# bitlayer-org/tap-stark

Hardware: AMD Instinct MI355X
Metric: trace cells/sec (proofs/sec alongside), 2^20x64 BabyBear trace (higher is better)
Workload: dtype u32

## Files before the change

### tap-stark_amd/csrc/kernels.hpp

```cpp
#pragma once
#include <stdint.h>

#include "bb.hpp"
#include "context.hpp"
#include "ntt_plan.hpp"

namespace ts {

struct ColMat {
    uint32_t* d = nullptr;
    uint64_t height = 0;
    uint32_t width = 0;
    uint64_t col_stride = 0;
};

void launch_build_twiddles(Context& ctx, uint32_t* W, uint32_t* Winv, unsigned log_size);
void launch_build_shift_tables(Context& ctx, uint32_t* lo, uint32_t* hi, uint32_t n_hi,
                               uint32_t n_cosets, uint32_t shift_mont, unsigned log_N,
                               unsigned log_blowup, uint32_t scale_mont);
const uint32_t* coset_scale_table(Context& ctx, unsigned log_n, unsigned log_blowup, uint32_t shift);
void launch_transpose_bitrev(Context& ctx, const uint32_t* src, uint32_t* dst, unsigned log_n,
                             uint32_t w, uint64_t dst_col_stride, uint32_t src_width = 0);
bool launch_transpose_bitrev_r16(Context& ctx, const uint32_t* src, uint32_t* dst, unsigned log_n, uint32_t w,
                                 uint64_t dst_col_stride, uint32_t src_width = 0);
void launch_transpose_plain(Context& ctx, const uint32_t* src, uint32_t* dst, uint64_t n, uint32_t w,
                            uint64_t dst_col_stride);
void launch_transpose_to_row_major(Context& ctx, const uint32_t* src, uint64_t col_stride,
                                   uint32_t* dst, uint64_t h, uint32_t w);
void launch_transpose_unbitrev(Context& ctx, const uint32_t* src, uint64_t col_stride, uint32_t* dst,
                               unsigned log_h, uint32_t w);
void coset_lde(Context& ctx, uint32_t* evals, uint64_t in_col_stride, uint32_t ncols, unsigned log_n,
               unsigned log_blowup, uint32_t shift, uint32_t* out, uint64_t out_col_stride,
               uint32_t beta0 = 0, uint32_t n_beta = 0, bool first_round_done = false,
               uint32_t* evals2 = nullptr, uint32_t shift2 = 0, uint32_t gw = 0, bool stage_timers = true);

inline void ntt_require_shape(const NttPlan& p, uint32_t ncols, uint64_t stride_a, uint64_t stride_b, bool lde) {
    if (const char* why = ntt_plan_refusal(p, ncols, stride_a, stride_b, lde)) throw Error(TS_ERR_INVALID, why);
}
void launch_contig_inverse(Context& ctx, const NttPlan& p, uint32_t* data, uint64_t col_stride, uint32_t ncols,
                           bool first_round_done = false, uint32_t* data2 = nullptr, uint32_t gw = 0xffffffffu);
void launch_contig_forward(Context& ctx, const NttPlan& p, uint32_t* data, uint64_t col_stride, uint32_t ncols,
                           uint32_t n_blocks);

void dft_columns(Context& ctx, uint32_t* cols, uint64_t col_stride, uint32_t ncols, unsigned log_n, bool inverse,
                 uint32_t shift);
void dft_batch(Context& ctx, const uint32_t* in, uint32_t* out, unsigned log_n, uint32_t w, bool inverse,
               uint32_t shift);
void coset_lde_batch(Context& ctx, const uint32_t* in, uint32_t* out, unsigned log_n, uint32_t w, unsigned added_bits,
                     uint32_t shift, bool bit_reversed);
void launch_bit_reverse_rows(Context& ctx, const uint32_t* src, uint32_t* dst, unsigned log_h, uint32_t w);

constexpr int MAX_BATCH_MATS = 64;
struct LeafMats {
    const uint32_t* d[MAX_BATCH_MATS];
    uint64_t col_stride[MAX_BATCH_MATS];
    uint32_t width[MAX_BATCH_MATS];
    uint8_t row_shift[MAX_BATCH_MATS];
    uint32_t n_mats;
    uint32_t total_width;
    const uint32_t* const* cols;
};
void launch_leaf_hash(Context& ctx, const LeafMats& mats, uint64_t height, uint32_t* digests);
void launch_leaf_hash_ef_pairs(Context& ctx, const uint32_t* vec, uint64_t n_rows, uint32_t* digests);
struct DevChallenger;
bool launch_merkle_levels(Context& ctx, uint32_t* tree, unsigned log_leaves,
                          DevChallenger* ch = nullptr, uint32_t* root_out = nullptr,
                          Ef* beta_out = nullptr);
void launch_merkle_tree_from(Context& ctx, uint32_t* tree, unsigned log_leaves, unsigned first_level,
                             DevChallenger* ch, uint32_t* root_out, Ef* beta_out);
bool leaf_tree_enabled(unsigned log_leaves);
void launch_commit_tree(Context& ctx, const LeafMats& mats, unsigned log_leaves, uint32_t* tree,
                        uint32_t* root_out = nullptr);
void launch_shard_top(Context& ctx, const uint32_t* subroots, uint32_t G, uint32_t* top,
                      DevChallenger* ch, uint32_t* root_out, Ef* beta_out);
void launch_merkle_one_level(Context& ctx, const uint32_t* children, uint32_t* parents,
                             uint64_t n_parents);
void launch_merkle_inject(Context& ctx, uint32_t* nodes, const uint32_t* inj, uint64_t n);
inline uint64_t merkle_level_offset(unsigned log_leaves, unsigned level) {
    uint64_t off = 0;
    for (unsigned l = 0; l < level; l++) off += (uint64_t)1 << (log_leaves - l);
    return off;
}
inline uint64_t merkle_total_digests(unsigned log_leaves) { return ((uint64_t)2 << log_leaves) - 1; }

struct AirProgram;
const uint32_t* selector_table(Context& ctx, unsigned log_n, unsigned log_qd, uint32_t shift);
constexpr int MAX_QUOTIENT_CHUNKS = 64;
struct QuotOut {
    uint32_t* chunk[MAX_QUOTIENT_CHUNKS];
};
void launch_quotient(Context& ctx, const AirProgram& air, const ColMat& trace_lde, unsigned log_n,
                     unsigned log_qd, const uint32_t* d_consts_mont, const uint32_t* d_alpha_pows_mont,
                     const QuotOut& out, uint64_t row_begin = 0, uint64_t row_end = 0,
                     uint32_t shift = GENERATOR, const ColMat* prep_lde = nullptr);
void launch_chunk_mix(Context& ctx, uint32_t* const* d_chunk_ptrs, uint32_t qd, uint64_t rows, uint64_t col_stride,
                      const uint32_t* d_mix_mont);

void launch_check_constraints(Context& ctx, const AirProgram& air, const uint32_t* trace_row_major,
                              uint64_t n, const uint32_t* d_consts_mont,
                              unsigned long long* d_violation, const uint32_t* prep_row_major = nullptr);

void launch_bary_weights(Context& ctx, unsigned log_n, const Ef* points_mont, uint32_t n_points,
                         Ef* out, uint32_t coset_gen = 0);
struct BaryPending {
    DevBuf<uint32_t> partial[3];
    uint32_t* out[3] = {nullptr, nullptr, nullptr};
    uint32_t n_blocks[3] = {0, 0, 0}, n_words[3] = {0, 0, 0};
    uint32_t n = 0, capacity = 2;
};
void launch_bary_dots(Context& ctx, const ColMat& m, unsigned log_n, const Ef* weights,
                      uint32_t n_points, Ef* out, BaryPending* pending = nullptr);
void launch_bary_finish(Context& ctx, BaryPending& pending);
struct ReduceArgs {
    Ef z_mont[2];
    Ef off_mont[2];
    Ef rys[2];
    uint32_t n_points;
    uint32_t accumulate;
};
void launch_reduce(Context& ctx, const ColMat& m, unsigned log_h, const uint32_t* d_alpha_pows_mont,
                   const ReduceArgs& args, Ef* ro);
struct FusedReduceArgs {
    Ef z_mont[2];
    Ef off_t[2];
    Ef k0, k1;
    const uint32_t* chunk_w;
    const uint32_t* chunk[MAX_QUOTIENT_CHUNKS];
    uint64_t chunk_stride;
    uint32_t n_chunks;
    uint64_t row0, rows;
};
void launch_reduce_fused(Context& ctx, const ColMat& trace, unsigned log_h,
                         const uint32_t* d_alpha_pows_mont, const FusedReduceArgs& args, Ef* ro,
                         const ColMat* prep = nullptr, const Ef* prep_off_mont = nullptr);
void launch_reduce_low(Context& ctx, const ColMat& trace, unsigned log_n, const uint32_t* d_alpha_pows_mont,
                       const FusedReduceArgs& args, const Ef* weights, uint32_t* out);
void launch_ef_interleave(Context& ctx, const uint32_t* cols, uint64_t col_stride, uint64_t rows, Ef* out);

void launch_fri_fold(Context& ctx, const Ef* in, uint64_t h, Ef beta_canonical, Ef* out,
                     uint32_t* next_digests);
void launch_fri_fold_dev(Context& ctx, const Ef* in, uint64_t h, const Ef* d_beta, Ef* out,
                         uint32_t* next_digests, uint64_t h_global = 0, uint64_t row0 = 0);
struct FriRoundLaunch {
    const Ef* prev = nullptr;
    const Ef* d_beta_prev = nullptr;
    Ef* cur = nullptr;
    uint64_t h = 0;
    uint32_t* tree = nullptr;
    DevChallenger* ch = nullptr;
    uint32_t* root_out = nullptr;
    Ef* beta_out = nullptr;
    uint64_t h_global = 0, row0 = 0;
};
void launch_fri_commit_round(Context& ctx, const FriRoundLaunch& r);
constexpr int FRI_TAIL_LOG = 10;
constexpr uint32_t FRI_POW_NONE = 0xffffffffu;
void launch_fri_tail(Context& ctx, const Ef* in, uint32_t L0, uint32_t blowup, DevChallenger* ch,
                     Ef* tail_vecs, uint32_t* tail_trees, uint32_t* roots_out, Ef* betas_out,
                     Ef* final_out, uint32_t pow_bits = 0, uint32_t* pow_out = nullptr,
                     const Ef* beta_in = nullptr);
void launch_vec_add(Context& ctx, Ef* acc, const Ef* other, uint64_t n);
struct FriGatherDesc {
    const uint32_t* vec;
    const uint32_t* tree;
    uint32_t log_leaves;
    uint32_t shift;
    uint64_t out_vals;
    uint64_t out_path;
};
struct RowGatherJob {
    LeafMats mats;
    uint32_t shift;
    uint32_t pad;
    uint64_t out;
};
void launch_gather_queries(Context& ctx, const RowGatherJob* d_rows, uint32_t n_rows, uint32_t max_row_width,
                           const FriGatherDesc* d_descs, uint32_t n_descs, uint32_t max_log_leaves,
                           const uint32_t* d_indices, uint32_t n_idx, uint32_t* out);

double alu_ceiling(Context& ctx, int kind);
double bench_stage(Context& ctx, int stage, unsigned log_n, uint32_t width, unsigned log_blowup, uint32_t reps);

void launch_trace_fibonacci(Context& ctx, uint32_t* out, uint32_t a, uint32_t b, uint64_t n);
void launch_trace_synth_mul(Context& ctx, uint32_t* out, uint64_t n, uint32_t width, uint64_t seed);
void launch_trace_synth_ext(Context& ctx, uint32_t* out, uint64_t n, uint32_t width, uint64_t seed);

enum : uint8_t { COL_U32 = 0, COL_U16 = 1, COL_U8 = 2, COL_MONTY32 = 3, COL_MONTY31 = 4 };
struct IngestPlan {
    bool planar = false;
    uint64_t height = 0;
    uint32_t width = 0;
    uint64_t stride = 0;
    uint64_t bytes = 0;
    int uniform4 = -1;
    std::vector<uint64_t> table;
};
IngestPlan ingest_plan(const uint8_t* kinds, uint32_t n_kinds, bool planar, uint64_t row_stride, uint64_t height,
                       uint32_t width);
void launch_ingest(Context& ctx, const IngestPlan& plan, const uint8_t* src, uint32_t* out);
void launch_scale_words(Context& ctx, const uint32_t* in, uint32_t* out, uint64_t n, uint32_t mult);
uint32_t monty_ingest_factor(uint32_t kind);

}
```

### tap-stark_amd/csrc/ntt_dft.hip

```cpp
#include <algorithm>

#include "ntt_rounds.hpp"

namespace ts {

constexpr int DFT_LO_BITS = 10;

__device__ __forceinline__ uint32_t dft_factor(const uint32_t* __restrict__ lo, const uint32_t* __restrict__ hi,
                                               uint32_t k) {
    return mont_mul(lo[k & ((1u << DFT_LO_BITS) - 1)], hi[k >> DFT_LO_BITS]);
}

template <bool INV, bool SCALE, int PLAN, int TILE = TILE_ELEMS, int NTM = NT_MID>
__global__ void __launch_bounds__(NTM)
k_dft_mid(uint32_t* data, uint64_t col_stride, unsigned log_len, unsigned log_T, unsigned row_shift,
          const uint32_t* __restrict__ W, const uint32_t* __restrict__ f_lo, const uint32_t* __restrict__ f_hi) {
    __shared__ uint32_t s[padded(TILE)];
    constexpr int PER_THREAD = TILE / NTM;
    if (PLAN == 1) {
        log_len = 8;
        log_T = 5;
    }
    const uint32_t j2_0 = blockIdx.x << log_T;
    uint32_t* g = data + (uint64_t)blockIdx.y * col_stride + j2_0;
    const uint32_t total = 1u << (log_len + log_T);
    const uint32_t tmask = (1u << log_T) - 1;
    auto off = [&](uint32_t i) { return ((i >> log_T) << row_shift) + (i & tmask); };
    if constexpr (PLAN == 1) {
        uint32_t t[PER_THREAD];
#pragma unroll
        for (int k = 0; k < PER_THREAD; k++) t[k] = g[off(threadIdx.x + (uint32_t)k * NTM)];
#pragma unroll
        for (int k = 0; k < PER_THREAD; k++) {
            const uint32_t i = threadIdx.x + (uint32_t)k * NTM;
            if (!INV && SCALE) t[k] = mont_mul_lazy(t[k], dft_factor(f_lo, f_hi, off(i) + j2_0));
            s[pad(i)] = t[k];
        }
    } else {
        for (uint32_t i = threadIdx.x; i < total; i += NTM) {
            uint32_t v = g[off(i)];
            if (!INV && SCALE) v = mont_mul_lazy(v, dft_factor(f_lo, f_hi, off(i) + j2_0));
            s[pad(i)] = v;
        }
    }
    __syncthreads();
    if constexpr (PLAN == 1) {
        if (!INV) {
            radix_round<4, false, 9, NTM, true>(s, 13, 0, 0, 0, W);
            radix_round<4, false, 5, NTM>(s, 13, 4, 0, 0, W);
        } else {
            radix_round<4, true, 5, NTM>(s, 13, 4, 0, 0, W);
            radix_round<4, true, 9, NTM, true>(s, 13, 0, 0, 0, W);
        }
    } else {
        if (!INV) tile_forward_rt<NTM>(s, log_len, log_T, 0, 0, W);
        else tile_inverse_rt<NTM>(s, log_len, log_T, 0, 0, W);
    }
    auto finish = [&](uint32_t v, uint32_t i) {
        if (INV) return SCALE ? mont_mul(v, dft_factor(f_lo, f_hi, off(i) + j2_0)) : red2p(v);
        return row_shift != 0 ? v : red2p(v);
    };
    if constexpr (PLAN == 1) {
        uint32_t t[PER_THREAD];
#pragma unroll
        for (int k = 0; k < PER_THREAD; k++) t[k] = s[pad(threadIdx.x + (uint32_t)k * NTM)];
#pragma unroll
        for (int k = 0; k < PER_THREAD; k++) {
            const uint32_t i = threadIdx.x + (uint32_t)k * NTM;
            g[off(i)] = finish(t[k], i);
        }
    } else {
        for (uint32_t i = threadIdx.x; i < total; i += NTM) g[off(i)] = finish(s[pad(i)], i);
    }
}

__global__ void __launch_bounds__(256)
k_bit_reverse_rows(const uint32_t* __restrict__ src, uint32_t* __restrict__ dst, unsigned log_h, uint32_t w) {
    const uint64_t idx = ((uint64_t)blockIdx.y * gridDim.x + blockIdx.x) * 256 + threadIdx.x;
    const uint64_t r = idx / w;
    if (r >> log_h) return;
    const uint32_t c = (uint32_t)(idx - r * w);
    dst[idx] = src[(uint64_t)bitrev32((uint32_t)r, log_h) * w + c];
}

void launch_bit_reverse_rows(Context& ctx, const uint32_t* src, uint32_t* dst, unsigned log_h, uint32_t w) {
    const uint64_t blocks = ((((uint64_t)w) << log_h) + 255) / 256;
    const uint32_t gx = (uint32_t)std::min<uint64_t>(blocks, 1u << 20);
    TS_LAUNCH(ctx, k_bit_reverse_rows, dim3(gx, (uint32_t)((blocks + gx - 1) / gx)), dim3(256), 0, src, dst, log_h, w);
    TS_HIP(hipGetLastError());
}

template <bool INV, bool SCALE>
static void launch_dft_mid_of(Context& ctx, const NttPlan& p, uint32_t* cols, uint64_t col_stride, uint32_t ncols,
                              const uint32_t* f_lo, const uint32_t* f_hi, const char* const (&names)[3]) {
    const uint32_t* W = INV ? ctx.d_twiddle_inv : ctx.d_twiddle_fwd;
    auto launch = [&](auto kernel) {
        TS_LAUNCH_NAMED(ctx, names[(int)p.mid], kernel, dim3(p.tiles, ncols), dim3(NT_MID), 0, cols, col_stride,
                        p.log_len, p.log_T, p.row_shift, W, f_lo, f_hi);
    };
    if (p.mid == NttMid::TILE16384) launch(k_dft_mid<INV, SCALE, 0, 16384>);
    else if (p.mid == NttMid::FIXED256) launch(k_dft_mid<INV, SCALE, 1>);
    else launch(k_dft_mid<INV, SCALE, 0>);
}

static void launch_dft_mid(Context& ctx, const NttPlan& p, uint32_t* cols, uint64_t col_stride, uint32_t ncols,
                           bool inverse, bool scale, const uint32_t* f_lo, const uint32_t* f_hi) {
    if (inverse)
        launch_dft_mid_of<true, true>(ctx, p, cols, col_stride, ncols, f_lo, f_hi,
                                      {"(k_dft_mid<true, true, 0>)", "(k_dft_mid<true, true, 1>)",
                                       "(k_dft_mid<true, true, 0, 16384>)"});
    else if (scale)
        launch_dft_mid_of<false, true>(ctx, p, cols, col_stride, ncols, f_lo, f_hi,
                                       {"(k_dft_mid<false, true, 0>)", "(k_dft_mid<false, true, 1>)",
                                        "(k_dft_mid<false, true, 0, 16384>)"});
    else
        launch_dft_mid_of<false, false>(ctx, p, cols, col_stride, ncols, f_lo, f_hi,
                                        {"(k_dft_mid<false, false, 0>)", "(k_dft_mid<false, false, 1>)",
                                         "(k_dft_mid<false, false, 0, 16384>)"});
}

void dft_columns(Context& ctx, uint32_t* cols, uint64_t col_stride, uint32_t ncols, unsigned log_n, bool inverse,
                 uint32_t shift) {
    if (ncols == 0) return;
    TS_REQUIRE(shift != 0 && shift < P, TS_ERR_INVALID, "dft: the coset shift must be in [1, p)");
    const NttPlan p = ntt_plan(log_n);
    ntt_require_shape(p, ncols, col_stride, 0, false);
    ctx.ensure_twiddles(log_n == 0 ? 1 : log_n);

    const bool scale = inverse || shift != 1;
    DevBuf<uint32_t> lo, hi;
    if (scale) {
        const uint32_t n_hi = log_n > (unsigned)DFT_LO_BITS ? 1u << (log_n - DFT_LO_BITS) : 1u;
        lo = DevBuf<uint32_t>(&ctx, 1u << DFT_LO_BITS);
        hi = DevBuf<uint32_t>(&ctx, n_hi);
        const uint32_t n_inv = inv_canon((uint32_t)((1ull << log_n) % P));
        launch_build_shift_tables(ctx, lo.p, hi.p, n_hi, 1, to_mont(inverse ? inv_canon(shift) : shift), log_n, 0,
                                  inverse ? to_mont(n_inv) : R_MOD_P);
    }
    if (inverse) {
        if (p.two_pass) launch_contig_inverse(ctx, p, cols, col_stride, ncols);
        launch_dft_mid(ctx, p, cols, col_stride, ncols, true, true, lo.p, hi.p);
    } else {
        launch_dft_mid(ctx, p, cols, col_stride, ncols, false, scale, lo.p, hi.p);
        if (p.two_pass) launch_contig_forward(ctx, p, cols, col_stride, ncols, 1);
    }
    TS_HIP(hipGetLastError());
}

void dft_batch(Context& ctx, const uint32_t* in, uint32_t* out, unsigned log_n, uint32_t w, bool inverse,
               uint32_t shift) {
    const uint64_t n = 1ull << log_n;
    DevBuf<uint32_t> cols(&ctx, (size_t)w * n);
    if (inverse) {
        launch_transpose_bitrev(ctx, in, cols.p, log_n, w, n);
        dft_columns(ctx, cols.p, n, w, log_n, true, shift);
        launch_transpose_to_row_major(ctx, cols.p, n, out, n, w);
    } else {
        launch_transpose_plain(ctx, in, cols.p, n, w, n);
        dft_columns(ctx, cols.p, n, w, log_n, false, shift);
        launch_transpose_unbitrev(ctx, cols.p, n, out, log_n, w);
    }
}

void coset_lde_batch(Context& ctx, const uint32_t* in, uint32_t* out, unsigned log_n, uint32_t w, unsigned added_bits,
                     uint32_t shift, bool bit_reversed) {
    const uint64_t n = 1ull << log_n, N = n << added_bits;
    DevBuf<uint32_t> cols(&ctx, (size_t)w * n), lde(&ctx, (size_t)w * N);
    const bool r16 = launch_transpose_bitrev_r16(ctx, in, cols.p, log_n, w, n);
    if (!r16) launch_transpose_bitrev(ctx, in, cols.p, log_n, w, n);
    coset_lde(ctx, cols.p, n, w, log_n, added_bits, shift, lde.p, N, 0, 0, r16);
    if (bit_reversed) launch_transpose_to_row_major(ctx, lde.p, N, out, N, w);
    else launch_transpose_unbitrev(ctx, lde.p, N, out, log_n + added_bits, w);
}

}
```

### tap-stark_amd/csrc/ntt_lde.hip

```cpp
#include <optional>
#include <type_traits>

#include "ntt_rounds.hpp"

namespace ts {

template <int LM, bool SKIP_R16 = false>
__global__ void __launch_bounds__(chunk_threads(LM))
k_intt_contig(uint32_t* __restrict__ data, uint64_t col_stride, unsigned log_n,
              const uint32_t* __restrict__ Winv, uint32_t* __restrict__ data2, uint32_t gw) {
    __shared__ uint32_t s[padded(1 << LM)];
    const uint32_t c = blockIdx.x;
    uint32_t* col = blockIdx.y < gw ? data + (uint64_t)blockIdx.y * col_stride
                                    : data2 + (uint64_t)(blockIdx.y - gw) * col_stride;
    uint32_t* g = col + ((uint64_t)c << LM);
    chunk_load<LM>(s, g);
    chunk_rounds<LM, true, SKIP_R16>(s, log_n - LM, c, Winv);
    chunk_store<LM, false>(s, g);
}

__global__ void __launch_bounds__(256)
k_transpose_bitrev_r16(const uint32_t* __restrict__ src, uint32_t* __restrict__ dst, unsigned log_n,
                       uint32_t w, uint64_t dst_col_stride, uint32_t src_width,
                       const uint32_t* __restrict__ Winv) {
    __shared__ uint32_t tile[64][65];
    const uint32_t p0 = blockIdx.x << 6;
    const uint32_t c0 = blockIdx.y * 64;
    const uint32_t tx = threadIdx.x & 63, ty = threadIdx.x >> 6;
    const uint32_t rb = bitrev32(p0, log_n);
    const uint64_t row_step = (uint64_t)src_width << (log_n - 6);
    uint32_t v[16];
    if (c0 + tx < w) {
        const uint32_t* sp = src + (uint64_t)rb * src_width + c0 + tx;
#pragma unroll
        for (int q = 0; q < 16; q++) v[q] = sp[(uint64_t)(__brev(16 * ty + (uint32_t)q) >> 26) * row_step];
    } else {
#pragma unroll
        for (int q = 0; q < 16; q++) v[q] = 0;
    }
    radix_butterflies<4, true, false>(v, log_n - 4, 0, 0, (p0 >> 4) + ty, Winv);
#pragma unroll
    for (int q = 0; q < 16; q++) tile[16 * ty + q][tx] = v[q];
    __syncthreads();
    uint32_t t[16];
#pragma unroll
    for (int k = 0; k < 16; k++) t[k] = tile[tx][ty + 4 * k];
    uint32_t* dp = dst + (uint64_t)(c0 + ty) * dst_col_stride + p0 + tx;
#pragma unroll
    for (int k = 0; k < 16; k++)
        if (c0 + ty + 4 * k < w) dp[(uint64_t)(4 * k) * dst_col_stride] = t[k];
}

template <int LM, int CPW = 1>
__global__ void __launch_bounds__(chunk_threads(LM), CPW > 1 ? 4 : 1)
k_lde_fwd_contig(uint32_t* __restrict__ out, uint64_t out_col_stride, unsigned log_n,
                 const uint32_t* __restrict__ W) {
    __shared__ uint32_t s[padded(1 << LM)];
    constexpr int NT = chunk_threads(LM);
    constexpr int NV = (1 << LM) / 4 / NT;
    const uint32_t beta = blockIdx.z;
    uint32_t* col = out + (uint64_t)blockIdx.y * out_col_stride + ((uint64_t)beta << log_n);
    if constexpr (CPW == 1) {
        const uint32_t c = blockIdx.x;
        uint32_t* o = col + ((uint64_t)c << LM);
        chunk_load<LM>(s, o);
        chunk_rounds<LM, false>(s, log_n - LM, c, W);
        chunk_store<LM, true>(s, o);
    } else {
        const uint32_t c0 = blockIdx.x * CPW;
        uint4 v[NV];
        {
            const uint4* g4 = reinterpret_cast<const uint4*>(col + ((uint64_t)c0 << LM));
#pragma unroll
            for (int k = 0; k < NV; k++) v[k] = g4[threadIdx.x + (uint32_t)k * NT];
        }
#pragma unroll 1
        for (int i = 0; i < CPW; i++) {
            const uint32_t c = c0 + i;
#pragma unroll
            for (int k = 0; k < NV; k++) {
                const uint32_t i4 = threadIdx.x + (uint32_t)k * NT;
                const uint32_t a = 4 * i4 + (i4 >> 3);
                s[a] = v[k].x;
                s[a + 1] = v[k].y;
                s[a + 2] = v[k].z;
                s[a + 3] = v[k].w;
            }
            __syncthreads();
            if (i + 1 < CPW) {
                const uint4* g4 = reinterpret_cast<const uint4*>(col + ((uint64_t)(c + 1) << LM));
#pragma unroll
                for (int k = 0; k < NV; k++) v[k] = g4[threadIdx.x + (uint32_t)k * NT];
            }
            chunk_rounds<LM, false>(s, log_n - LM, c, W);
            chunk_store<LM, true>(s, col + ((uint64_t)c << LM));
            __syncthreads();
        }
    }
}

template <int PLAN, int TILE = TILE_ELEMS, int NTM = NT_MID, int LM = LOG_M>
__global__ void __launch_bounds__(NTM)
k_lde_mid(const uint32_t* __restrict__ evals, uint64_t in_col_stride, uint32_t* __restrict__ out,
          uint64_t out_col_stride, unsigned log_n, unsigned log_len, unsigned log_T,
          unsigned row_shift, unsigned beta0, unsigned n_cosets, const uint32_t* __restrict__ W,
          const uint32_t* __restrict__ Winv, const uint32_t* __restrict__ scale_a,
          const uint32_t* __restrict__ evals2, const uint32_t* __restrict__ scale_b, uint32_t gw) {
    __shared__ uint32_t s[padded(TILE)];
    constexpr int PER_THREAD = TILE / NTM;
    if (PLAN == 1) {
        log_len = 8;
        log_T = 5;
    }
    const bool remap = PLAN == 0 && log_T < 5 && gridDim.x >= 8;
    uint32_t bx = remap ? (blockIdx.x & 7) * (gridDim.x >> 3) + (blockIdx.x >> 3) : blockIdx.x;
    uint32_t col_id = blockIdx.y;
    if constexpr (PLAN == 1) {
        const uint32_t ncols = gridDim.x >> (LM - 5);
        bx = (blockIdx.x & 31) + 32 * (blockIdx.x / (32 * ncols));
        col_id = (blockIdx.x >> 5) % ncols;
    }
    const uint32_t j2_0 = bx << log_T;
    const uint32_t* g = (col_id < gw ? evals + (uint64_t)col_id * in_col_stride
                                     : evals2 + (uint64_t)(col_id - gw) * in_col_stride) + j2_0;
    const uint32_t* __restrict__ scale = col_id < gw ? scale_a : scale_b;
    const uint32_t total = 1u << (log_len + log_T);
    const uint32_t tmask = (1u << log_T) - 1;
    if constexpr (PLAN == 1) {
        uint32_t t[PER_THREAD];
#pragma unroll
        for (int k = 0; k < PER_THREAD; k++) {
            const uint32_t i = threadIdx.x + (uint32_t)k * NTM;
            t[k] = g[((uint64_t)(i >> log_T) << row_shift) + (i & tmask)];
        }
#pragma unroll
        for (int k = 0; k < PER_THREAD; k++) s[pad(threadIdx.x + (uint32_t)k * NTM)] = t[k];
    } else {
        for (uint32_t i = threadIdx.x; i < total; i += NTM)
            s[pad(i)] = g[((uint64_t)(i >> log_T) << row_shift) + (i & tmask)];
    }
    __syncthreads();
    if (PLAN == 1) {
        radix_round<4, true, 5, NTM>(s, 13, 4, 0, 0, Winv);
    } else {
        tile_inverse_rt<NTM>(s, log_len, log_T, 0, 0, Winv);
    }
    uint32_t coef[PER_THREAD];
#pragma unroll
    for (int k = 0; k < PER_THREAD; k++) {
        const uint32_t i = threadIdx.x + (uint32_t)k * NTM;
        coef[k] = i < total ? s[pad(i)] : 0u;
    }
    constexpr int GP = PER_THREAD / 16;
    if constexpr (PLAN == 1) {
#pragma unroll
        for (int j = 0; j < GP; j++) {
            uint32_t v[16];
#pragma unroll
            for (int q = 0; q < 16; q++) v[q] = coef[j + GP * q];
            radix_butterflies<4, true, true>(v, 0, 0, 0, 0, Winv);
#pragma unroll
            for (int q = 0; q < 16; q++) coef[j + GP * q] = v[q];
        }
    }
    constexpr bool PREFETCH = PLAN == 1;
    uint32_t scv[PREFETCH ? 16 : 1];
    const uint32_t* scp = nullptr;
    if constexpr (PREFETCH) {
        const uint32_t i0 = threadIdx.x;
        scp = scale + ((uint64_t)(i0 >> 5) << LM) + (i0 & 31) + j2_0;
#pragma unroll
        for (int q = 0; q < 16; q++)
            scv[q] = (scp + ((uint64_t)beta0 << log_n))[(uint64_t)q * (NTM >> 5) << LM];
    }
    for (uint32_t bl = 0; bl < n_cosets; bl++) {
        const uint32_t beta = beta0 + bl;
        const uint32_t* sc = scale + ((uint64_t)beta << log_n);
        __syncthreads();
        if constexpr (PLAN == 1) {
#pragma unroll
            for (int j = 0; j < GP; j++) {
                uint32_t v[16];
#pragma unroll
                for (int q = 0; q < 16; q++) v[q] = mont_mul_lazy(coef[j + GP * q], scv[q]);
                if (bl + 1 < n_cosets) {
                    const uint32_t* nx = scp + ((uint64_t)(beta + 1) << log_n);
#pragma unroll
                    for (int q = 0; q < 16; q++) scv[q] = nx[(uint64_t)q * (NTM >> 5) << LM];
                }
                radix_butterflies<4, false, true>(v, 0, 0, 0, 0, W);
#pragma unroll
                for (int q = 0; q < 16; q++) s[pad(threadIdx.x + (uint32_t)(j + GP * q) * NTM)] = v[q];
            }
            __syncthreads();
            uint32_t* og = out + (uint64_t)col_id * out_col_stride + ((uint64_t)bl << log_n) + j2_0;
            radix_round<4, false, 5, NTM>(s, 13, 4, 0, 0, W);
            uint32_t t[PER_THREAD];
#pragma unroll
            for (int k = 0; k < PER_THREAD; k++) t[k] = s[pad(threadIdx.x + (uint32_t)k * NTM)];
            uint32_t* ot = og + ((uint64_t)(threadIdx.x >> 5) << LM) + (threadIdx.x & 31);
#pragma unroll
            for (int k = 0; k < PER_THREAD; k++) ot[(uint64_t)k * (NTM >> 5) << LM] = t[k];
            continue;
        } else {
#pragma unroll
            for (int k = 0; k < PER_THREAD; k++) {
                const uint32_t i = threadIdx.x + (uint32_t)k * NTM;
                if (i < total) {
                    const uint32_t kk = ((i >> log_T) << row_shift) + (i & tmask) + j2_0;
                    s[pad(i)] = mont_mul_lazy(coef[k], sc[kk]);
                }
            }
            __syncthreads();
            tile_forward_rt<NTM>(s, log_len, log_T, 0, 0, W);
        }
        uint32_t* o = out + (uint64_t)col_id * out_col_stride + ((uint64_t)bl << log_n) + j2_0;
        if (row_shift != 0) {
            for (uint32_t i = threadIdx.x; i < total; i += NTM)
                o[((uint64_t)(i >> log_T) << row_shift) + (i & tmask)] = s[pad(i)];
        } else {
            for (uint32_t i = threadIdx.x; i < total; i += NTM)
                o[((uint64_t)(i >> log_T) << row_shift) + (i & tmask)] = red2p(s[pad(i)]);
        }
    }
}

constexpr const char* INTT_NAME[3] = {"k_intt_contig<12>", "k_intt_contig<13>", "k_intt_contig<14>"};
constexpr const char* INTT_R16_NAME[3] = {"(k_intt_contig<12, true>)", "(k_intt_contig<13, true>)",
                                          "(k_intt_contig<14, true>)"};
constexpr const char* FWD_NAME[3] = {"k_lde_fwd_contig<12>", "k_lde_fwd_contig<13>", "(k_lde_fwd_contig<14, 4>)"};

template <class F>
static void with_chunk_log(unsigned LM, F&& f) {
    if (LM == 12) f(std::integral_constant<int, 12>{});
    else if (LM == 13) f(std::integral_constant<int, 13>{});
    else f(std::integral_constant<int, 14>{});
}

bool launch_transpose_bitrev_r16(Context& ctx, const uint32_t* src, uint32_t* dst, unsigned log_n, uint32_t w,
                                 uint64_t dst_col_stride, uint32_t src_width) {
    if (w == 0 || !ntt_plan(log_n).fused_first_round) return false;
    ctx.ensure_twiddles(log_n);
    TS_LAUNCH(ctx, k_transpose_bitrev_r16, dim3(1u << (log_n - 6), (w + 63) / 64), dim3(256), 0, src, dst, log_n, w,
              dst_col_stride, src_width ? src_width : w, (const uint32_t*)ctx.d_twiddle_inv);
    TS_HIP(hipGetLastError());
    return true;
}

void launch_contig_inverse(Context& ctx, const NttPlan& p, uint32_t* data, uint64_t col_stride, uint32_t ncols,
                           bool first_round_done, uint32_t* data2, uint32_t gw) {
    const uint32_t* Winv = ctx.d_twiddle_inv;
    with_chunk_log(p.LM, [&](auto lm) {
        constexpr int LM = decltype(lm)::value;
        const dim3 g(p.chunks, ncols), b(chunk_threads(LM));
        if (first_round_done)
            TS_LAUNCH_NAMED(ctx, INTT_R16_NAME[LM - 12], (k_intt_contig<LM, true>), g, b, 0, data, col_stride, p.log_n,
                            Winv, data2, gw);
        else
            TS_LAUNCH_NAMED(ctx, INTT_NAME[LM - 12], k_intt_contig<LM>, g, b, 0, data, col_stride, p.log_n, Winv, data2,
                            gw);
    });
}

static void launch_lde_mid(Context& ctx, const NttPlan& p, const uint32_t* evals, uint64_t in_col_stride,
                           uint32_t* out, uint64_t out_col_stride, uint32_t ncols, uint32_t beta0, uint32_t n_beta,
                           const uint32_t* scale, const uint32_t* evals2, const uint32_t* scale2, uint32_t gw) {
    const uint32_t *W = ctx.d_twiddle_fwd, *Winv = ctx.d_twiddle_inv;
    const dim3 grid(p.tiles, ncols), b(NT_MID);
    const dim3 grid1(p.tiles * ncols);
#define TS_MID_ARGS \
    evals, in_col_stride, out, out_col_stride, p.log_n, p.log_len, p.log_T, p.row_shift, beta0, n_beta, W, Winv, scale, \
        evals2, scale2, gw
    if (p.mid == NttMid::TILE16384)
        TS_LAUNCH_NAMED(ctx, "(k_lde_mid<0, 16384>)", (k_lde_mid<0, 16384>), grid, b, 0, TS_MID_ARGS);
    else if (p.mid == NttMid::FIXED256 && p.LM == 12)
        TS_LAUNCH_NAMED(ctx, "k_lde_mid<1>", k_lde_mid<1>, grid1, b, 0, TS_MID_ARGS);
    else if (p.mid == NttMid::FIXED256 && p.LM == 13)
        TS_LAUNCH_NAMED(ctx, "(k_lde_mid<1, 8192, 512, 13>)", (k_lde_mid<1, 8192, 512, 13>), grid1, b, 0, TS_MID_ARGS);
    else if (p.mid == NttMid::FIXED256)
        TS_LAUNCH_NAMED(ctx, "(k_lde_mid<1, 8192, 512, 14>)", (k_lde_mid<1, 8192, 512, 14>), grid1, b, 0, TS_MID_ARGS);
    else
        TS_LAUNCH_NAMED(ctx, "k_lde_mid<0>", k_lde_mid<0>, grid, b, 0, TS_MID_ARGS);
#undef TS_MID_ARGS
}

void launch_contig_forward(Context& ctx, const NttPlan& p, uint32_t* data, uint64_t col_stride, uint32_t ncols,
                           uint32_t n_blocks) {
    const uint32_t* W = ctx.d_twiddle_fwd;
    with_chunk_log(p.LM, [&](auto lm) {
        constexpr int LM = decltype(lm)::value;
        constexpr int CPW = LM == 14 ? 4 : 1;
        TS_LAUNCH_NAMED(ctx, FWD_NAME[LM - 12], (k_lde_fwd_contig<LM, CPW>), dim3(p.chunks / CPW, ncols, n_blocks),
                        dim3(chunk_threads(LM)), 0, data, col_stride, p.log_n, W);
    });
}

void coset_lde(Context& ctx, uint32_t* evals, uint64_t in_col_stride, uint32_t ncols, unsigned log_n,
               unsigned log_blowup, uint32_t shift, uint32_t* out, uint64_t out_col_stride,
               uint32_t beta0, uint32_t n_beta, bool first_round_done, uint32_t* evals2, uint32_t shift2,
               uint32_t gw, bool stage_timers) {
    if (ncols == 0) return;
    TS_REQUIRE(evals2 == nullptr || (gw >= 1 && gw < ncols && shift2 != 0), TS_ERR_INVALID,
               "coset_lde: second matrix needs its first column and its shift");
    if (evals2 == nullptr) gw = 0xffffffffu;
    TS_REQUIRE(log_n + log_blowup <= 27, TS_ERR_INVALID, "coset_lde: log_n + log_blowup > 27");
    const NttPlan p = ntt_plan(log_n);
    ntt_require_shape(p, ncols, in_col_stride, out_col_stride, true);
    TS_REQUIRE(!first_round_done || p.fused_first_round, TS_ERR_INVARIANT,
               "coset_lde: no contiguous inverse pass at this size");
    ctx.ensure_twiddles(log_n == 0 ? 1 : log_n);

    const uint32_t n_cosets = 1u << log_blowup;
    if (n_beta == 0) n_beta = n_cosets - beta0;
    TS_REQUIRE(beta0 < n_cosets && n_beta <= n_cosets - beta0, TS_ERR_INVALID, "coset_lde: coset range");
    const uint32_t* scale = coset_scale_table(ctx, log_n, log_blowup, shift);
    const uint32_t* scale2 = evals2 ? coset_scale_table(ctx, log_n, log_blowup, shift2) : nullptr;

    if (!p.two_pass) {
        launch_lde_mid(ctx, p, evals, in_col_stride, out, out_col_stride, ncols, beta0, n_beta, scale, evals2, scale2,
                       gw);
    } else {
        if (ctx.lde_pass_mask & 1u) {
            std::optional<StageTimer> t;
            if (stage_timers) t.emplace(&ctx, "lde: inverse NTT, contiguous stages");
            launch_contig_inverse(ctx, p, evals, in_col_stride, ncols, first_round_done, evals2, gw);
        }
        std::optional<StageTimer> t_rest;
        if (stage_timers) t_rest.emplace(&ctx, "lde: strided pass + forward NTT of the owned cosets");
        if (ctx.lde_pass_mask & 2u)
            launch_lde_mid(ctx, p, evals, in_col_stride, out, out_col_stride, ncols, beta0, n_beta, scale, evals2,
                           scale2, gw);
        if (ctx.lde_pass_mask & 4u) launch_contig_forward(ctx, p, out, out_col_stride, ncols, n_beta);
    }
    TS_HIP(hipGetLastError());
}

}
```

### tap-stark_amd/csrc/ntt_plan.hpp

```cpp
#pragma once
#include <stdint.h>

namespace ts {

constexpr int LOG_M = 12;
constexpr int TILE_ELEMS = 8192;
constexpr uint32_t NTT_MAX_COLS = 65535;

inline unsigned lde_chunk_log(unsigned log_n) {
    return (log_n == 21 || log_n == 22) ? log_n - 8 : (unsigned)LOG_M;
}

enum class NttMid {
    GENERIC,
    FIXED256,
    TILE16384,
};

struct NttPlan {
    unsigned log_n;
    unsigned LM;
    bool two_pass;
    unsigned sA;
    unsigned log_T;
    unsigned log_len;
    unsigned row_shift;
    NttMid mid;
    bool fused_first_round;
    uint32_t chunks;
    uint32_t tiles;
};

inline NttPlan ntt_plan(unsigned log_n) {
    NttPlan p{};
    p.log_n = log_n;
    p.LM = lde_chunk_log(log_n);
    p.two_pass = log_n > p.LM;
    p.sA = p.two_pass ? log_n - p.LM : 0;
    if (p.sA > 14) return p;
    if (p.two_pass && p.sA <= 13)
        while ((1u << (p.sA + p.log_T + 1)) <= (unsigned)TILE_ELEMS && p.log_T < 6) p.log_T++;
    p.log_len = p.two_pass ? p.sA : log_n;
    p.row_shift = p.two_pass ? p.LM : 0;
    p.mid = p.sA == 14 ? NttMid::TILE16384 : (p.sA == 8 && p.log_T == 5) ? NttMid::FIXED256 : NttMid::GENERIC;
    p.fused_first_round = p.two_pass;
    p.chunks = 1u << p.sA;
    p.tiles = p.two_pass ? 1u << (p.LM - p.log_T) : 1u;
    return p;
}

inline const char* ntt_plan_refusal(const NttPlan& p, uint32_t ncols, uint64_t stride_a, uint64_t stride_b, bool lde) {
    if (ncols > NTT_MAX_COLS) return lde ? "coset_lde: bad column count" : "dft: more than 65535 columns";
    if (p.sA > 14) return lde ? "coset_lde: log_n > 26" : "dft: height above 2^26";
    if (p.two_pass && (stride_a % 4 != 0 || stride_b % 4 != 0))
        return lde ? "coset_lde: column strides must be multiples of 4 elements"
                   : "dft: column stride must be a multiple of 4 elements";
    return nullptr;
}

}
```

Measured before the change: 25.02 billion.

## Skip computing the LDE coset that equals the original domain and copy evals

When the coset shift lies in the evaluation subgroup, one of the LDE cosets coincides with the input domain. This change detects that coset on the host, copies the input evaluations straight into its output slot, and skips it in both the strided mid pass and the contiguous forward pass. The goal is to remove one coset's worth of NTT work and writes. It adds an extra copy kernel, forces the non-r16 transpose path whenever the skip applies, and the detection only fires for shifts inside the subgroup, which typical generator shifts are not.

```diff
diff --git a/tap-stark_amd/csrc/kernels.hpp b/tap-stark_amd/csrc/kernels.hpp
--- a/tap-stark_amd/csrc/kernels.hpp
+++ b/tap-stark_amd/csrc/kernels.hpp
@@ -34,13 +34,17 @@
                uint32_t beta0 = 0, uint32_t n_beta = 0, bool first_round_done = false,
                uint32_t* evals2 = nullptr, uint32_t shift2 = 0, uint32_t gw = 0, bool stage_timers = true);
 
+constexpr uint32_t LDE_NO_OWN = 0xffffffffu;
+int lde_own_coset_used(unsigned log_n, unsigned log_blowup, uint32_t shift);
+
 inline void ntt_require_shape(const NttPlan& p, uint32_t ncols, uint64_t stride_a, uint64_t stride_b, bool lde) {
     if (const char* why = ntt_plan_refusal(p, ncols, stride_a, stride_b, lde)) throw Error(TS_ERR_INVALID, why);
 }
 void launch_contig_inverse(Context& ctx, const NttPlan& p, uint32_t* data, uint64_t col_stride, uint32_t ncols,
                            bool first_round_done = false, uint32_t* data2 = nullptr, uint32_t gw = 0xffffffffu);
 void launch_contig_forward(Context& ctx, const NttPlan& p, uint32_t* data, uint64_t col_stride, uint32_t ncols,
-                           uint32_t n_blocks);
+                           uint32_t n_blocks, uint32_t gw = 0xffffffffu, uint32_t own_a = LDE_NO_OWN,
+                           uint32_t own_b = LDE_NO_OWN);
 
 void dft_columns(Context& ctx, uint32_t* cols, uint64_t col_stride, uint32_t ncols, unsigned log_n, bool inverse,
                  uint32_t shift);
diff --git a/tap-stark_amd/csrc/ntt_dft.hip b/tap-stark_amd/csrc/ntt_dft.hip
--- a/tap-stark_amd/csrc/ntt_dft.hip
+++ b/tap-stark_amd/csrc/ntt_dft.hip
@@ -166,7 +166,8 @@
                      uint32_t shift, bool bit_reversed) {
     const uint64_t n = 1ull << log_n, N = n << added_bits;
     DevBuf<uint32_t> cols(&ctx, (size_t)w * n), lde(&ctx, (size_t)w * N);
-    const bool r16 = launch_transpose_bitrev_r16(ctx, in, cols.p, log_n, w, n);
+    const bool r16 = lde_own_coset_used(log_n, added_bits, shift) < 0 &&
+                     launch_transpose_bitrev_r16(ctx, in, cols.p, log_n, w, n);
     if (!r16) launch_transpose_bitrev(ctx, in, cols.p, log_n, w, n);
     coset_lde(ctx, cols.p, n, w, log_n, added_bits, shift, lde.p, N, 0, 0, r16);
     if (bit_reversed) launch_transpose_to_row_major(ctx, lde.p, N, out, N, w);
diff --git a/tap-stark_amd/csrc/ntt_lde.hip b/tap-stark_amd/csrc/ntt_lde.hip
--- a/tap-stark_amd/csrc/ntt_lde.hip
+++ b/tap-stark_amd/csrc/ntt_lde.hip
@@ -1,3 +1,5 @@
+#include <stdlib.h>
+
 #include <optional>
 #include <type_traits>
 
@@ -51,14 +53,12 @@
         if (c0 + ty + 4 * k < w) dp[(uint64_t)(4 * k) * dst_col_stride] = t[k];
 }
 
-template <int LM, int CPW = 1>
-__global__ void __launch_bounds__(chunk_threads(LM), CPW > 1 ? 4 : 1)
-k_lde_fwd_contig(uint32_t* __restrict__ out, uint64_t out_col_stride, unsigned log_n,
-                 const uint32_t* __restrict__ W) {
+template <int LM, int CPW>
+__device__ __forceinline__ void lde_fwd_contig_block(uint32_t* __restrict__ out, uint64_t out_col_stride, unsigned log_n,
+                                                     const uint32_t* __restrict__ W, const uint32_t beta) {
     __shared__ uint32_t s[padded(1 << LM)];
     constexpr int NT = chunk_threads(LM);
     constexpr int NV = (1 << LM) / 4 / NT;
-    const uint32_t beta = blockIdx.z;
     uint32_t* col = out + (uint64_t)blockIdx.y * out_col_stride + ((uint64_t)beta << log_n);
     if constexpr (CPW == 1) {
         const uint32_t c = blockIdx.x;
@@ -99,13 +99,29 @@
     }
 }
 
-template <int PLAN, int TILE = TILE_ELEMS, int NTM = NT_MID, int LM = LOG_M>
+template <int LM, int CPW = 1>
+__global__ void __launch_bounds__(chunk_threads(LM), CPW > 1 ? 4 : 1)
+k_lde_fwd_contig(uint32_t* __restrict__ out, uint64_t out_col_stride, unsigned log_n,
+                 const uint32_t* __restrict__ W) {
+    lde_fwd_contig_block<LM, CPW>(out, out_col_stride, log_n, W, blockIdx.z);
+}
+
+template <int LM, int CPW = 1>
+__global__ void __launch_bounds__(chunk_threads(LM), CPW > 1 ? 4 : 1)
+k_lde_fwd_contig_own(uint32_t* __restrict__ out, uint64_t out_col_stride, unsigned log_n,
+                     const uint32_t* __restrict__ W, uint32_t gw, uint32_t own_a, uint32_t own_b) {
+    const uint32_t own = blockIdx.y < gw ? own_a : own_b;
+    lde_fwd_contig_block<LM, CPW>(out, out_col_stride, log_n, W, blockIdx.z + (blockIdx.z >= own ? 1u : 0u));
+}
+
+template <int PLAN, int TILE = TILE_ELEMS, int NTM = NT_MID, int LM = LOG_M, bool OWN = false>
 __global__ void __launch_bounds__(NTM)
 k_lde_mid(const uint32_t* __restrict__ evals, uint64_t in_col_stride, uint32_t* __restrict__ out,
           uint64_t out_col_stride, unsigned log_n, unsigned log_len, unsigned log_T,
           unsigned row_shift, unsigned beta0, unsigned n_cosets, const uint32_t* __restrict__ W,
           const uint32_t* __restrict__ Winv, const uint32_t* __restrict__ scale_a,
-          const uint32_t* __restrict__ evals2, const uint32_t* __restrict__ scale_b, uint32_t gw) {
+          const uint32_t* __restrict__ evals2, const uint32_t* __restrict__ scale_b, uint32_t gw,
+          uint32_t own_a, uint32_t own_b) {
     __shared__ uint32_t s[padded(TILE)];
     constexpr int PER_THREAD = TILE / NTM;
     if (PLAN == 1) {
@@ -124,6 +140,7 @@
     const uint32_t* g = (col_id < gw ? evals + (uint64_t)col_id * in_col_stride
                                      : evals2 + (uint64_t)(col_id - gw) * in_col_stride) + j2_0;
     const uint32_t* __restrict__ scale = col_id < gw ? scale_a : scale_b;
+    const uint32_t own = OWN ? (col_id < gw ? own_a : own_b) : 0xffffffffu;
     const uint32_t total = 1u << (log_len + log_T);
     const uint32_t tmask = (1u << log_T) - 1;
     if constexpr (PLAN == 1) {
@@ -169,11 +186,13 @@
     if constexpr (PREFETCH) {
         const uint32_t i0 = threadIdx.x;
         scp = scale + ((uint64_t)(i0 >> 5) << LM) + (i0 & 31) + j2_0;
+        const uint32_t first = OWN && own == 0 ? 1u : 0u;
 #pragma unroll
         for (int q = 0; q < 16; q++)
-            scv[q] = (scp + ((uint64_t)beta0 << log_n))[(uint64_t)q * (NTM >> 5) << LM];
+            scv[q] = (scp + ((uint64_t)(beta0 + first) << log_n))[(uint64_t)q * (NTM >> 5) << LM];
     }
     for (uint32_t bl = 0; bl < n_cosets; bl++) {
+        if (OWN && bl == own) continue;
         const uint32_t beta = beta0 + bl;
         const uint32_t* sc = scale + ((uint64_t)beta << log_n);
         __syncthreads();
@@ -183,8 +202,9 @@
                 uint32_t v[16];
 #pragma unroll
                 for (int q = 0; q < 16; q++) v[q] = mont_mul_lazy(coef[j + GP * q], scv[q]);
-                if (bl + 1 < n_cosets) {
-                    const uint32_t* nx = scp + ((uint64_t)(beta + 1) << log_n);
+                const uint32_t nb = OWN && bl + 1 == own ? bl + 2 : bl + 1;
+                if (nb < n_cosets) {
+                    const uint32_t* nx = scp + ((uint64_t)(beta0 + nb) << log_n);
 #pragma unroll
                     for (int q = 0; q < 16; q++) scv[q] = nx[(uint64_t)q * (NTM >> 5) << LM];
                 }
@@ -222,6 +242,29 @@
             for (uint32_t i = threadIdx.x; i < total; i += NTM)
                 o[((uint64_t)(i >> log_T) << row_shift) + (i & tmask)] = red2p(s[pad(i)]);
         }
+    }
+}
+
+template <bool VEC>
+__global__ void __launch_bounds__(256)
+k_lde_own_copy(const uint32_t* __restrict__ evals, uint64_t in_col_stride, uint32_t* __restrict__ out,
+               uint64_t out_col_stride, unsigned log_n, const uint32_t* __restrict__ evals2, uint32_t gw,
+               uint32_t own_a, uint32_t own_b) {
+    const uint32_t col = blockIdx.y;
+    const uint32_t* src = col < gw ? evals + (uint64_t)col * in_col_stride
+                                   : evals2 + (uint64_t)(col - gw) * in_col_stride;
+    uint32_t* dst = out + (uint64_t)col * out_col_stride + ((uint64_t)(col < gw ? own_a : own_b) << log_n);
+    if constexpr (VEC) {
+        const uint4* s4 = reinterpret_cast<const uint4*>(src) + (uint64_t)blockIdx.x * 1024 + threadIdx.x;
+        uint4* d4 = reinterpret_cast<uint4*>(dst) + (uint64_t)blockIdx.x * 1024 + threadIdx.x;
+        uint4 v[4];
+#pragma unroll
+        for (int k = 0; k < 4; k++) v[k] = s4[256 * k];
+#pragma unroll
+        for (int k = 0; k < 4; k++) d4[256 * k] = v[k];
+    } else {
+        const uint64_t i = (uint64_t)blockIdx.x * 256 + threadIdx.x;
+        if (i < (1ull << log_n)) dst[i] = src[i];
     }
 }
 
@@ -264,14 +307,25 @@
 
 static void launch_lde_mid(Context& ctx, const NttPlan& p, const uint32_t* evals, uint64_t in_col_stride,
                            uint32_t* out, uint64_t out_col_stride, uint32_t ncols, uint32_t beta0, uint32_t n_beta,
-                           const uint32_t* scale, const uint32_t* evals2, const uint32_t* scale2, uint32_t gw) {
+                           const uint32_t* scale, const uint32_t* evals2, const uint32_t* scale2, uint32_t gw,
+                           uint32_t own_a, uint32_t own_b) {
     const uint32_t *W = ctx.d_twiddle_fwd, *Winv = ctx.d_twiddle_inv;
     const dim3 grid(p.tiles, ncols), b(NT_MID);
     const dim3 grid1(p.tiles * ncols);
 #define TS_MID_ARGS \
     evals, in_col_stride, out, out_col_stride, p.log_n, p.log_len, p.log_T, p.row_shift, beta0, n_beta, W, Winv, scale, \
-        evals2, scale2, gw
-    if (p.mid == NttMid::TILE16384)
+        evals2, scale2, gw, own_a, own_b
+    if (own_a != LDE_NO_OWN && p.mid == NttMid::FIXED256 && p.LM == 12)
+        TS_LAUNCH_NAMED(ctx, "k_lde_mid<1>", (k_lde_mid<1, TILE_ELEMS, NT_MID, 12, true>), grid1, b, 0, TS_MID_ARGS);
+    else if (own_a != LDE_NO_OWN && p.mid == NttMid::FIXED256 && p.LM == 13)
+        TS_LAUNCH_NAMED(ctx, "(k_lde_mid<1, 8192, 512, 13>)", (k_lde_mid<1, 8192, 512, 13, true>), grid1, b, 0,
+                        TS_MID_ARGS);
+    else if (own_a != LDE_NO_OWN && p.mid == NttMid::FIXED256)
+        TS_LAUNCH_NAMED(ctx, "(k_lde_mid<1, 8192, 512, 14>)", (k_lde_mid<1, 8192, 512, 14, true>), grid1, b, 0,
+                        TS_MID_ARGS);
+    else if (own_a != LDE_NO_OWN)
+        TS_LAUNCH_NAMED(ctx, "k_lde_mid<0>", (k_lde_mid<0, TILE_ELEMS, NT_MID, LOG_M, true>), grid, b, 0, TS_MID_ARGS);
+    else if (p.mid == NttMid::TILE16384)
         TS_LAUNCH_NAMED(ctx, "(k_lde_mid<0, 16384>)", (k_lde_mid<0, 16384>), grid, b, 0, TS_MID_ARGS);
     else if (p.mid == NttMid::FIXED256 && p.LM == 12)
         TS_LAUNCH_NAMED(ctx, "k_lde_mid<1>", k_lde_mid<1>, grid1, b, 0, TS_MID_ARGS);
@@ -285,14 +339,25 @@
 }
 
 void launch_contig_forward(Context& ctx, const NttPlan& p, uint32_t* data, uint64_t col_stride, uint32_t ncols,
-                           uint32_t n_blocks) {
+                           uint32_t n_blocks, uint32_t gw, uint32_t own_a, uint32_t own_b) {
     const uint32_t* W = ctx.d_twiddle_fwd;
     with_chunk_log(p.LM, [&](auto lm) {
         constexpr int LM = decltype(lm)::value;
         constexpr int CPW = LM == 14 ? 4 : 1;
-        TS_LAUNCH_NAMED(ctx, FWD_NAME[LM - 12], (k_lde_fwd_contig<LM, CPW>), dim3(p.chunks / CPW, ncols, n_blocks),
-                        dim3(chunk_threads(LM)), 0, data, col_stride, p.log_n, W);
+        if (own_a != LDE_NO_OWN)
+            TS_LAUNCH_NAMED(ctx, FWD_NAME[LM - 12], (k_lde_fwd_contig_own<LM, CPW>),
+                            dim3(p.chunks / CPW, ncols, n_blocks - 1), dim3(chunk_threads(LM)), 0, data, col_stride,
+                            p.log_n, W, gw, own_a, own_b);
+        else
+            TS_LAUNCH_NAMED(ctx, FWD_NAME[LM - 12], (k_lde_fwd_contig<LM, CPW>), dim3(p.chunks / CPW, ncols, n_blocks),
+                            dim3(chunk_threads(LM)), 0, data, col_stride, p.log_n, W);
     });
+}
+
+int lde_own_coset_used(unsigned log_n, unsigned log_blowup, uint32_t shift) {
+    if (const char* e = getenv("TS_LDE_OWN_COSET"); e && *e && atoi(e) == 0) return -1;
+    if (log_blowup == 0 || log_n + log_blowup > 27 || ntt_plan(log_n).mid == NttMid::TILE16384) return -1;
+    return lde_own_coset(log_n, log_blowup, shift);
 }
 
 void coset_lde(Context& ctx, uint32_t* evals, uint64_t in_col_stride, uint32_t ncols, unsigned log_n,
@@ -316,9 +381,28 @@
     const uint32_t* scale = coset_scale_table(ctx, log_n, log_blowup, shift);
     const uint32_t* scale2 = evals2 ? coset_scale_table(ctx, log_n, log_blowup, shift2) : nullptr;
 
+    uint32_t own_a = LDE_NO_OWN, own_b = LDE_NO_OWN;
+    if (beta0 == 0 && n_beta == n_cosets && !first_round_done && ctx.lde_pass_mask == 7u) {
+        const int a = lde_own_coset_used(log_n, log_blowup, shift);
+        const int b = evals2 ? lde_own_coset_used(log_n, log_blowup, shift2) : a;
+        if (a >= 0 && b >= 0) {
+            own_a = (uint32_t)a;
+            own_b = (uint32_t)b;
+            const uint64_t n = 1ull << log_n;
+            if (p.two_pass)
+                TS_LAUNCH_NAMED(ctx, "k_lde_own_copy", k_lde_own_copy<true>, dim3((unsigned)(n >> 12), ncols), dim3(256), 0,
+                                (const uint32_t*)evals, in_col_stride, out, out_col_stride, log_n,
+                                (const uint32_t*)evals2, gw, own_a, own_b);
+            else
+                TS_LAUNCH_NAMED(ctx, "k_lde_own_copy", k_lde_own_copy<false>, dim3((unsigned)((n + 255) / 256), ncols),
+                                dim3(256), 0, (const uint32_t*)evals, in_col_stride, out, out_col_stride, log_n,
+                                (const uint32_t*)evals2, gw, own_a, own_b);
+        }
+    }
+
     if (!p.two_pass) {
         launch_lde_mid(ctx, p, evals, in_col_stride, out, out_col_stride, ncols, beta0, n_beta, scale, evals2, scale2,
-                       gw);
+                       gw, own_a, own_b);
     } else {
         if (ctx.lde_pass_mask & 1u) {
             std::optional<StageTimer> t;
@@ -329,8 +413,8 @@
         if (stage_timers) t_rest.emplace(&ctx, "lde: strided pass + forward NTT of the owned cosets");
         if (ctx.lde_pass_mask & 2u)
             launch_lde_mid(ctx, p, evals, in_col_stride, out, out_col_stride, ncols, beta0, n_beta, scale, evals2,
-                           scale2, gw);
-        if (ctx.lde_pass_mask & 4u) launch_contig_forward(ctx, p, out, out_col_stride, ncols, n_beta);
+                           scale2, gw, own_a, own_b);
+        if (ctx.lde_pass_mask & 4u) launch_contig_forward(ctx, p, out, out_col_stride, ncols, n_beta, gw, own_a, own_b);
     }
     TS_HIP(hipGetLastError());
 }
diff --git a/tap-stark_amd/csrc/ntt_plan.hpp b/tap-stark_amd/csrc/ntt_plan.hpp
--- a/tap-stark_amd/csrc/ntt_plan.hpp
+++ b/tap-stark_amd/csrc/ntt_plan.hpp
@@ -1,5 +1,7 @@
 #pragma once
 #include <stdint.h>
+
+#include "bb.hpp"
 
 namespace ts {
 
@@ -58,4 +60,15 @@
     return nullptr;
 }
 
+inline int lde_own_coset(unsigned log_n, unsigned log_blowup, uint32_t shift) {
+    const unsigned log_N = log_n + log_blowup;
+    if (log_N > 27 || shift == 0 || shift >= P) return -1;
+    if (pow_canon(shift, 1ull << log_N) != 1u) return -1;
+    const uint32_t w = to_mont(two_adic_generator(log_N));
+    uint32_t s = shift;
+    for (uint32_t e = 0; e < (1u << log_blowup); e++, s = mont_mul(s, w))
+        if (s == 1u) return (int)bitrev32(e, log_blowup);
+    return -1;
 }
+
+}
```

Result: faster. 25.39 billion, median of 6 (+1.4%).
